# Rutgers-ECE-MML4SS/multimodal-sensor-fusion-with-attention-RajeevAtla

Measured on AMD Instinct MI355X. Metric: HybridFusion fwd+bwd samples/sec at 1/2/4/8 MI355X; CPU-ref parity, higher is better.
Workload: dtype fp32; 1 GPU; c2: HybridFusion M=3 B=256/gpu L=128 D=128 H=128 heads=4 C=5 dropout=0.1 train, fwd+CE(ls=0.05)+bwd+clip(1.0)+AdamW; fused step (flat buffers, one hipGraph); global_batch=256, per_gpu_batch=256, seq_len=128, parallelism=dp1, graph=True, matmul_precision=highest

## Files before the change

multimodal-sensor-fusion-with-attention-rajeevatla_amd/csrc/capi_util.h:

```cpp
#pragma once

#include <cstdarg>
#include <cstdio>
#include <cstring>
#include <string>
#include <vector>

#include "mmf_internal.h"
#include "mmfusion.h"

namespace mmf {

int fail(int code, const char* fmt, ...);

struct ProfRec { const char* name; hipEvent_t a, b; };
struct LaunchRec { const char* stage; const char* kernel; double flops, bytes; hipEvent_t a, b; };
struct Prof {
  bool on = false;
  const char* cur_stage = "";
  std::vector<ProfRec> recs;
  std::vector<LaunchRec> launches;
  std::vector<hipEvent_t> pool;
  size_t next = 0;
  hipEvent_t ev() {
    if (next == pool.size()) {
      hipEvent_t e;
      if (hipEventCreate(&e) != hipSuccess) return nullptr;
      pool.push_back(e);
    }
    return pool[next++];
  }
};
extern Prof g_prof;

// ... 79 lines not shown

inline void add_src(GemmJob& j, Operand a, Operand b, int K) {
  GemmSrc& s = j.src[j.nsrc++];
  s.a = a;
  s.b = b;
  s.K = K;
}

inline void split_rows(int rows, int& nsplit, int& kchunk, int hint = 0) {
  if (hint > 0) {
    kchunk = (rows + hint - 1) / hint;
    kchunk = (kchunk + 31) & ~31;
    nsplit = (rows + kchunk - 1) / kchunk;
    return;
  }
  int chunk = rows / 4;
  if (chunk > 512) chunk = 512;
  if (chunk < 64) chunk = 64;
  nsplit = (rows + chunk - 1) / chunk;
  if (nsplit < 1) nsplit = 1;
  if (nsplit > 64) nsplit = 64;
  kchunk = (rows + nsplit - 1) / nsplit;
  kchunk = (kchunk + 31) & ~31;
  nsplit = (rows + kchunk - 1) / kchunk;
}

inline size_t slab_bytes(int M, int N, int rows) {
  int nsplit, kchunk;
  split_rows(rows, nsplit, kchunk);
  return ((((size_t)nsplit * M * N * 4) + 255) & ~size_t(255)) +
         ((((size_t)nsplit * M * 4) + 255) & ~size_t(255)) + 256;
}

struct WgradPlan {
  std::vector<GemmJob> jobs;
  std::vector<ReduceJob> reds;
  int split_hint = 0;
  std::vector<GemmJob> jobs_b16;
  bool size_only = false;
};

inline void plan_wgrad(WgradPlan& wp, Bump& ws, int M, int N, int rows, Operand a, Operand b,
                       float* out_w, float* out_b, bool has_db, float alpha = 1.f) {
  int nsplit, kchunk;
  split_rows(rows, nsplit, kchunk, wp.split_hint);
  float* part = ws.take<float>((size_t)nsplit * M * N);
  float* part_db = has_db ? ws.take<float>((size_t)nsplit * M) : nullptr;
  GemmJob j = make_job(M, N, part, N, EPI_PARTIAL);
  j.g.alpha = alpha;
  j.g.nsplit = nsplit;
  j.g.kchunk = kchunk;
  j.g.part_db = part_db;
  if (wp.size_only) return;
  add_src(j, a, b, rows);
  wp.jobs.push_back(j);
  ReduceJob r;
  memset(&r, 0, sizeof(r));
  r.nbatch = 1;
  r.part = part;
  r.part_db = part_db;
  r.out = out_w;
  r.db = out_b;
  r.nsplit = nsplit;
  r.M = M;
  r.N = N;
  wp.reds.push_back(r);
}

inline void plan_wgrad_batched(WgradPlan& wp, Bump& ws, int M, int N, int rows, Operand a, Operand b,
                               float* out_w, int nbatch, int bs_a, int bs_b, int bs_out) {
  int nsplit, kchunk;
  split_rows(rows, nsplit, kchunk);
  float* part = ws.take<float>((size_t)nbatch * nsplit * M * N);
  GemmJob j = make_job(M, N, part, N, EPI_PARTIAL);
  j.g.nsplit = nsplit;
  j.g.kchunk = kchunk;
  j.g.nbatch = nbatch;
  j.g.bs_a = bs_a;
// ... 36 lines not shown
```

multimodal-sensor-fusion-with-attention-rajeevatla_amd/csrc/gemm.hip:

```cpp
#include <algorithm>
#include <cstdlib>
#include <cstring>
#include <map>
#include <vector>

#include "mmf_device.h"

namespace mmf {

namespace {

constexpr int BM = 128, BN = 128, BK = 32, NT = 256;
#ifndef MMF_GEMM_DK
#define MMF_GEMM_DK 16
#endif
#ifndef MMF_GEMM_NS
#define MMF_GEMM_NS 3
#endif
constexpr int LDS_STRIDE = BM + 4;
constexpr int LDS_STRIDE_T = BM + 1;

typedef float f32x4 __attribute__((ext_vector_type(4)));

struct TileCtx {
  int i0, j0, batch, split, nsplit;
  float* Cb;
  float* part_db;
  const float* biasb;
  int brs_off;
};

int gemm_interleave_mode() {
  const char* e = getenv("MMF_GEMM_ILV");
  if (!e || !e[0]) return 1;
  return e[0] == '0' ? 0 : (e[0] == '2' ? 2 : 1);
}
// ... 585 lines not shown
    __syncthreads();
    if (t >= BM) red[t - BM] = dbsum;
    __syncthreads();
    if (t < BM && T.i0 + t < G.M)
      T.part_db[(int64_t)T.split * G.M + T.i0 + t] = (dbsum + red[t]) * G.alpha;
  }
  if constexpr (WIDE) {
    f32x16 lo[2][2] = {{acc[0][0], acc[0][1]}, {acc[1][0], acc[1][1]}};
    epilogue<PR>(G, T, lo, lds, rs, p, inv_keep, wm, wn, h, c);
    TileCtx T2 = T;
    T2.j0 += BN;
    f32x16 hi[2][2] = {{acc[0][2], acc[0][3]}, {acc[1][2], acc[1][3]}};
    epilogue<PR>(G, T2, hi, lds, rs, p, inv_keep, wm, wn, h, c);
  } else {
    epilogue<PR>(G, T, acc, lds, rs, p, inv_keep, wm, wn, h, c);
  }
  if constexpr (!CHAIN) break;
  if (!G.chain) break;
  gi = G.chain - 1;
  asm volatile("s_waitcnt vmcnt(0)" ::: "memory");
  __syncthreads();
  __builtin_amdgcn_fence(__ATOMIC_ACQUIRE, "agent");
  }
}

template <int AMODE, int BMODE, int DK, int NSTAGE, int BF = 0, int B16 = 0, int WIDE = 0>
__global__ __launch_bounds__(NT, (NSTAGE * (B16 ? DK / 2 : DK) <= 32 ? 4 : 2)) void gemm_lds_kernel(const GemmArgs args) {
  gemm_lds_body<AMODE, BMODE, DK, NSTAGE, BF, B16, WIDE, 0>(args);
}
template <int AMODE, int BMODE, int DK, int NSTAGE, int BF = 0>
__global__ __launch_bounds__(NT) __attribute__((amdgpu_waves_per_eu(3)))
void gemm_lds_chain_kernel(const GemmArgs args) {
  gemm_lds_body<AMODE, BMODE, DK, NSTAGE, BF, 0, 0, 1>(args);
}

constexpr int WSR_DK = 16, WSR_NS = 6, WSR_NKC = 16;

template <int BF, bool EXT>
__global__ __launch_bounds__(NT, 2) void gemm_wsr_kernel(const GemmArgs args, int total_items, int K) {
  constexpr int DTILE = BM * WSR_DK;
  __shared__ __attribute__((aligned(16))) float ring[WSR_NS * DTILE];
  __shared__ float csx[BN];
  const int t = threadIdx.x;
  const int lane = t & 63, wave = t >> 6;
  const int h = lane >> 5, c = lane & 31;
  const int wm = wave >> 1, wn = wave & 1;
  const int nkt = K / WSR_DK, nkc = K / 8;

  RngSnap rs{0, 0};
  const float p = args.drop_p;
  const float inv_keep = p < 1.f ? 1.f / (1.f - p) : 0.f;
  const uint32_t thr = p16(p);
  if (p > 0.f && args.rng) rs = *args.rng;
  if (args.rng_advance && blockIdx.x == 0 && threadIdx.x == 0) args.rng_advance[1] += 1;
  const int nwg = gridDim.x;
  const int item0 = (int)(((int64_t)blockIdx.x * total_items) / nwg);
  const int item1 = (int)(((int64_t)(blockIdx.x + 1) * total_items) / nwg);
  if (item0 >= item1) return;

  const int nflat = (item1 - item0) * nkt;
  auto item_group = [&](int item, int& rowtile) {
    int g = 0;
#pragma unroll
    for (int i = 1; i < GEMM_MAX_GROUPS; ++i)
      if (i < args.ngroups && item >= args.tile_off[i]) g = i;
    rowtile = item - args.tile_off[g];
// ... 1018 lines not shown
        mmf_launch((KERNEL<MODE_KR, MODE_KR>), grid, dim3(NT), 0, st, args);       \
      else                                                                                 \
        mmf_launch((KERNEL<MODE_KR, MODE_RK>), grid, dim3(NT), 0, st, args);
      if (nch) {
        if (bmode == MODE_KR) {
          if (pr == 2) mmf_launch((gemm_lds_chain_kernel<MODE_RK, MODE_KR, 16, 3, 2>), grid, dim3(NT), 0, st, args);
          else if (pr == 1) mmf_launch((gemm_lds_chain_kernel<MODE_RK, MODE_KR, 16, 3, 1>), grid, dim3(NT), 0, st, args);
          else mmf_launch((gemm_lds_chain_kernel<MODE_RK, MODE_KR, 16, 3, 0>), grid, dim3(NT), 0, st, args);
        } else {
          if (pr == 2) mmf_launch((gemm_lds_chain_kernel<MODE_RK, MODE_RK, 16, 3, 2>), grid, dim3(NT), 0, st, args);
          else if (pr == 1) mmf_launch((gemm_lds_chain_kernel<MODE_RK, MODE_RK, 16, 3, 1>), grid, dim3(NT), 0, st, args);
          else mmf_launch((gemm_lds_chain_kernel<MODE_RK, MODE_RK, 16, 3, 0>), grid, dim3(NT), 0, st, args);
        }
      } else if (fast) {
        MMF_LAUNCH_CFG(MMF_GEMM_DK, MMF_GEMM_NS)
      } else {
        MMF_LAUNCH(gemm_generic_kernel)
      }
#undef MMF_LAUNCH
#undef MMF_LAUNCH_CFG
#undef MMF_LAUNCH_CFG2
      hipError_t e = hipGetLastError();
      if (e != hipSuccess) return e;
    } else if (args.rng_advance) {
      rng_advance = args.rng_advance;
    }
  }
  if (!later.empty())
    if (hipError_t e = launch_gemm(later.data(), (int)later.size(), amode, bmode, drop_p, rng, st, nullptr))
      return e;
  return left.finish(hipSuccess);
}

__global__ __launch_bounds__(256) void cvt_bf16_kernel(const CvtArgs a) {
  const int q = blockIdx.y;
  const float* s = a.src[q];
  __bf16* d = a.dst[q];
  const int64_t n = a.n[q];
  if (float* d32 = a.dst32[q]) {
    for (int64_t i = (int64_t)blockIdx.x * 256 + threadIdx.x; i < n; i += (int64_t)gridDim.x * 256) d32[i] = s[i];
    return;
  }
  for (int64_t i = 4 * ((int64_t)blockIdx.x * 256 + threadIdx.x); i < n; i += 4 * (int64_t)gridDim.x * 256) {
    if (i + 4 <= n) {
      const float4 v = *reinterpret_cast<const float4*>(s + i);
      d[i] = (__bf16)v.x; d[i + 1] = (__bf16)v.y; d[i + 2] = (__bf16)v.z; d[i + 3] = (__bf16)v.w;
    } else {
      for (int64_t e = i; e < n; ++e) d[e] = (__bf16)s[e];
    }
  }
}

hipError_t launch_cvt_bf16(const CvtArgs& a, hipStream_t st) {
  if (a.count <= 0) return hipSuccess;
  if (a.count > CVT_MAX) return hipErrorInvalidValue;
  int64_t mx = 0;
  double by = 0.0;
  for (int i = 0; i < a.count; ++i) {
    if (!a.dst32[i] && ((uintptr_t)a.src[i] & 15) != 0) return hipErrorInvalidValue;
    mx = std::max<int64_t>(mx, a.dst32[i] ? a.n[i] : a.n[i] / 4);
    by += (a.dst32[i] ? 8.0 : 6.0) * a.n[i];
  }
  const int gx = (int)std::min<int64_t>((mx + 255) / 256, 64);
  ProfLaunch prof_(st, "cvt_bf16_kernel", 0.0, by);
  mmf_launch(cvt_bf16_kernel, dim3(std::max(gx, 1), a.count), dim3(256), 0, st, a);
  return hipGetLastError();
// ... 269 lines not shown
```

multimodal-sensor-fusion-with-attention-rajeevatla_amd/csrc/hybrid.hip:

```cpp
#include <algorithm>
#include <cmath>
#include <cstdlib>
#include <cstdio>
#include <cstring>
#include <unistd.h>

#include "capi_util.h"

using namespace mmf;

namespace {

const char* const kPlanKnobs[] = {
    "MMF_PSTORE", "MMF_NO_LONG_FUSED", "MMF_NO_FUSED_BWD", "MMF_NO_BF16_QK", "MMF_NO_GEMM_B16",
    "MMF_QK_CAT", "MMF_NO_DQK_B16", "MMF_NO_PROJ_B16", "MMF_NO_PCOL", "MMF_NO_POOLE", "MMF_POOLE_FLAT",
    "MMF_NO_L1_LEAN", "MMF_WGRAD_SPLIT_CAP", "MMF_NO_SIDE_STREAM", "MMF_SIDE_STREAM", "MMF_KW_SERIAL",
    "MMF_KW_FUSED", "MMF_NO_KW_FUSED", "MMF_NO_GATE_B16", "MMF_POOL_PER_PAIR", "MMF_TAIL_S"};

uint32_t plan_flags_now() {
  uint32_t sum = 0;
  for (char** e = environ; e && *e; ++e) {
    const char* s = *e;
    if (std::strncmp(s, "MMF_", 4) != 0) continue;
    for (const char* k : kPlanKnobs) {
      const size_t n = std::strlen(k);
      if (std::strncmp(s, k, n) != 0 || s[n] != '=') continue;
      uint32_t h = 2166136261u;
      for (const char* c = s; *c; ++c) h = (h ^ (uint8_t)*c) * 16777619u;
      sum += h | 1u;
      break;
    }
  }
  return sum;
}

int check_buffers(const mmf_hybrid_desc* d, size_t need_saved, size_t need_ws) {
  const uint32_t now = plan_flags_now();
  if (d->plan_flags != now)
    return fail(MMF_EINVAL,
                "the plan switches (MMF_* environment) changed since this descriptor's buffers were sized "
                "(plan_flags %08x, now %08x): size the buffers again and set plan_flags = mmf_hybrid_plan_flags()",
                d->plan_flags, now);
  if (need_saved != ~size_t(0) && need_saved > d->saved_capacity)
    return fail(MMF_EINVAL, "saved buffer too small: this call's layout needs %zu bytes, saved_capacity is %llu",
                need_saved, (unsigned long long)d->saved_capacity);
  if (need_ws != ~size_t(0) && need_ws > d->workspace_capacity)
    return fail(MMF_EINVAL, "workspace too small: this call's layout needs %zu bytes, workspace_capacity is %llu",
                need_ws, (unsigned long long)d->workspace_capacity);
  return MMF_OK;
}
// ... 279 lines not shown
                d->num_heads);
  if (d->hidden % 4 != 0 || d->hidden > 1024)
    return fail(MMF_ELIMIT, "hidden_dim must be a multiple of 4 and <= 1024 (got %d)", d->hidden);
  if (d->num_classes < 1) return fail(MMF_EINVAL, "num_classes must be >= 1");
  if (d->num_pairs < 0 || d->num_pairs > d->num_modalities * (d->num_modalities - 1))
    return fail(MMF_EINVAL, "bad num_pairs %d", d->num_pairs);
  for (int m = 0; m < d->num_modalities; ++m) {
    if (d->in_dim[m] < 1) return fail(MMF_EINVAL, "in_dim[%d] must be >= 1", m);
    if (d->seq_len[m] < 0) return fail(MMF_EINVAL, "seq_len[%d] must be >= 0", m);
  }
  for (int g = 0; g < d->num_pairs; ++g) {
    const int q = d->pair_q[g], k = d->pair_k[g];
    if (q < 0 || k < 0 || q >= d->num_modalities || k >= d->num_modalities || q == k)
      return fail(MMF_EINVAL, "bad pair %d: (%d, %d)", g, q, k);
  }
  if (!(d->dropout >= 0.f && d->dropout < 1.f))
    return fail(MMF_EINVAL, "dropout must be in [0, 1) (got %g)", (double)d->dropout);
  for (int g = 0; g < d->num_pairs; ++g)
    if (wide_pair(d, g) && !wide_supported(d->batch, d->num_heads, Lm(d, d->pair_q[g]), Lm(d, d->pair_k[g])))
      return fail(MMF_ELIMIT, "head_dim %d: pair %d's (heads x Lq x Lk) score tensor is too large",
                  d->hidden / d->num_heads, g);
  return MMF_OK;
}

void plan_wgrads(const mmf_hybrid_desc* d, const float* const* x, const float* mask,
                 const float* dlogits, const Saved& s, const Ws& w, const mmf_hybrid_grads* G,
                 Bump& bw, WgradPlan& wp, int part = 0) {
  const bool want_pairs = part != 2, want_proj = part != 1;
  const int B = d->batch, M = d->num_modalities, H = d->hidden, C = d->num_classes;
  const int nh = d->num_heads, hd = H / nh;
  const bool pool = use_pool(d);
  static const mmf_hybrid_grads kNull = {};
  const mmf_hybrid_grads* g = G ? G : &kNull;
  const int kBigRows = 4096;
  int nbig = 0;
  for (int p = 0; p < d->num_pairs && want_pairs; ++p) {
    const int lq = Lm(d, d->pair_q[p]), lk = Lm(d, d->pair_k[p]);
    if (!pool) nbig += (B * lq >= kBigRows) + (B * lk >= kBigRows);
    if (!single_key(d, p)) nbig += (B * lq >= kBigRows) + (B * lk >= kBigRows);
  }
  for (int m = 0; m < M && want_proj; ++m) nbig += (B * Lm(d, m) >= kBigRows);
  const int slots = 3 * device_cu_count();
  const int rem = nbig % GEMM_MAX_GROUPS, nfull = nbig - rem;
  int bi = 0;
  auto hint = [&](int rows) {
    if (rows < kBigRows) return 0;
    const int per = bi++ < nfull ? GEMM_MAX_GROUPS : rem;
    int sp = slots / per;
    if (const char* e = getenv("MMF_WGRAD_SPLIT_CAP")) sp = std::min(sp, std::max(1, atoi(e)));
    return std::max(1, std::min(sp, 256));
  };
  if (want_pairs) {
    plan_wgrad(wp, bw, C, H, B, opnd(dlogits, C), opnd(s.h1, H), g->cls2.w, g->cls2.b);
    plan_wgrad(wp, bw, H, H, B, opnd(w.dz1, H), opnd(s.fused, H), g->cls1.w, g->cls1.b);
    for (int m = 0; m < M; ++m)
      plan_wgrad(wp, bw, 1, H, B, opnd(w.dscore ? w.dscore + m : nullptr, M),
                 opnd(s.pooled ? s.pooled + (size_t)m * H : nullptr, M * H), g->gate[m].w, g->gate[m].b);
  }
  for (int p = 0; p < d->num_pairs && want_pairs; ++p) {
    const int q = d->pair_q[p], k = d->pair_k[p];
    const int lq = Lm(d, q), lk = Lm(d, k);
    const float* cq = w.cvec ? w.cvec + (size_t)q * H : nullptr;
    if (pool) {
      plan_wgrad(wp, bw, H, H, B, opnd(cq, M * H), opnd(s.Ob[p], H), g->o[p].w, g->o[p].b);
      Operand dob = opnd(w.dOb[p], H), u = opnd(s.U[p], nh * H), rr = opnd(s.r[p], nh);
      dob.vec = u.vec = (hd % 4 == 0) && (H % 4 == 0);
      rr.vec = 0;
      plan_wgrad_batched(wp, bw, hd, H, B, dob, u, g->v[p].w, nh, hd, H, hd * H);
      plan_wgrad_batched(wp, bw, hd, 1, B, dob, rr, g->v[p].b, nh, hd, 1, hd);
    } else {
      wp.split_hint = hint(B * lq);
      plan_wgrad(wp, bw, H, H, B * lq, opnd(cq, M * H, lq), opnd(s.O[p], H), g->o[p].w, g->o[p].b,
                 1.f / (float)lq);
      wp.split_hint = hint(B * lk);
      plan_wgrad(wp, bw, H, H, B * lk, opnd(w.dV[p], H), opnd(s.P[k], H), g->v[p].w, g->v[p].b);
    }
    if (single_key(d, p)) {
      plan_zero(wp, H, H, g->q[p].w, g->q[p].b);
      plan_zero(wp, H, H, g->k[p].w, g->k[p].b);
      continue;
    }
    const bool b16 = dqk_b16_on(d);
    const float* pq = b16 ? reinterpret_cast<const float*>(s.Pb[q]) : s.P[q];
    const float* pk = b16 ? reinterpret_cast<const float*>(s.Pb[k]) : s.P[k];
    wp.split_hint = hint(B * lq);
    plan_wgrad(wp, bw, H, H, B * lq, opnd(w.dQ[p], s.ldq[p]), opnd(pq, H), g->q[p].w, g->q[p].b);
    if (b16 && !wp.size_only) { wp.jobs_b16.push_back(wp.jobs.back()); wp.jobs.pop_back(); }
    wp.split_hint = hint(B * lk);
    plan_wgrad(wp, bw, H, H, B * lk, opnd(w.dK[p], s.ldk[p]), opnd(pk, H), g->k[p].w, g->k[p].b);
    if (b16 && !wp.size_only) { wp.jobs_b16.push_back(wp.jobs.back()); wp.jobs.pop_back(); }
    wp.split_hint = 0;
  }
  for (int m = 0; m < M && want_proj; ++m) {
    const int L = Lm(d, m), D = d->in_dim[m];
    wp.split_hint = hint(B * L);
    plan_wgrad(wp, bw, H, D, B * L, opnd(w.dZ[m], H), opnd(s.Xd[m], D), g->proj[m].w, g->proj[m].b);
    if (proj_b16_on(d) && !wp.size_only) { wp.jobs_b16.push_back(wp.jobs.back()); wp.jobs.pop_back(); }
    wp.split_hint = 0;
  }
}

size_t saved_bytes(const mmf_hybrid_desc* d) {
  MathScope math_(d->matmul_precision);
  Bump bp(nullptr);
  Saved s{};
  layout_saved(d, bp, s);
  return bp.off + 256;
}

size_t workspace_bytes(const mmf_hybrid_desc* d) {
  MathScope math_(d->matmul_precision);
  Bump bs(nullptr);
  Saved s{};
  layout_saved(d, bs, s);
  Bump bw(nullptr);
  Ws w;
  layout_ws(d, bw, w);
  size_t top = 0;
  for (int part = 0; part < 3; ++part) {
    Bump b = bw;
    WgradPlan wp;
    wp.size_only = true;
    plan_wgrads(d, nullptr, nullptr, nullptr, s, w, nullptr, b, wp, part);
    top = std::max(top, b.off);
  }
  return top + 256;
}

void fill_head(HeadArgs& ha, const mmf_hybrid_desc* d, const mmf_hybrid_params* W, const float* mask,
               const Saved& s) {
  const bool pool = use_pool(d);
// ... 774 lines not shown
      for (int g = 0; g < d->num_pairs; ++g)
        if (d->pair_k[g] == m) {
          e.pbar[e.nsrc] = s.pbar[g];
          e.du[e.nsrc++] = w.dU[g];
        }
    }
    if (!em.empty()) STAGE_TRY("bwd.pool_e", launch_pool_e(em.data(), (int)em.size(), B, nh, H, st));
  } else if (d->num_pairs) {
    std::vector<GemmJob> jobs;
    for (int g = 0; g < d->num_pairs; ++g) {
      const int q = d->pair_q[g], lq = Lm(d, q);
      GemmJob j = make_job(B * lq, H, w.dO[g], H, 0);
      j.g.alpha = 1.f / (float)lq;
      add_src(j, opnd(w.cvec + (size_t)q * H, M * H, lq), opnd(W->o[g].w, H), H);
      jobs.push_back(j);
    }
    STAGE_TRY("bwd.out_dO_gemm", launch_gemm(jobs.data(), (int)jobs.size(), MODE_RK, MODE_KR, 0.f, rng, st));
    if (nmp) {
      STAGE_TRY("bwd.attn_prep", launch_attn_bwd_stage(0, pairs.data(), nmp, B, nh, hd, scale, p, rng, st));
      STAGE_TRY("bwd.attn_dkv", launch_attn_bwd_stage(1, pairs.data(), nmp, B, nh, hd, scale, p, rng, st));
      STAGE_TRY("bwd.attn_dq", launch_attn_bwd_stage(2, pairs.data(), nmp, B, nh, hd, scale, p, rng, st));
    }
    if (nsk) STAGE_TRY("bwd.attn_single_key_dv", launch_sk_dv(skp.data(), nsk, B, nh, hd, p, rng, st));
    if (nwp) STAGE_TRY("bwd.attn_wide", launch_wide_bwd(wpairs.data(), nwp, B, nh, hd, scale, p, rng, false, st));
  }
  }
  if (part == 1) {
    std::stable_sort(wp.jobs.begin(), wp.jobs.end(), [](const GemmJob& a, const GemmJob& b) {
      const int64_t wa = (int64_t)a.g.nsplit * std::max(1, a.g.nbatch) * a.g.M * a.g.N;
      const int64_t wb = (int64_t)b.g.nsplit * std::max(1, b.g.nbatch) * b.g.M * b.g.N;
      return wa > wb;
    });
    STAGE_TRY("bwd.wgrad_gemm", launch_gemm(wp.jobs.data(), (int)wp.jobs.size(), MODE_KR, MODE_KR, p, rng, st));
    if (!wp.jobs_b16.empty())
      STAGE_TRY("bwd.wgrad_gemm", launch_gemm_b16(wp.jobs_b16.data(), (int)wp.jobs_b16.size(), st, MODE_KR, MODE_KR));
    STAGE_TRY("bwd.wgrad_reduce", launch_reduce(wp.reds.data(), (int)wp.reds.size(), st));
    return MMF_OK;
  }
  std::vector<GemmJob> dxjobs(M);
  std::vector<bool> has_dx(M, false);
  const bool pb16 = proj_b16_on(d);
  for (int m = 0; m < M; ++m) {
    if (!dx || !dx[m]) continue;
    const int L = Lm(d, m), D = d->in_dim[m];
    GemmJob j = make_job(B * L, D, dx[m], D, EPI_ROWSCALE | (drop ? EPI_DROP : 0));
    j.g.rowscale = mask; j.g.rs_div = L; j.g.rs_stride = M; j.g.rs_off = m;
    j.g.drop_site = SITE_IN + m;
    add_src(j, opnd(w.dZ[m], H), opnd(pb16 ? reinterpret_cast<const float*>(s.Wpb[m]) : W->proj[m].w, D), H);
    dxjobs[m] = j;
    has_dx[m] = true;
  }
  const bool chain_dx = !dqk_b16_on(d) && !pb16 && getenv("MMF_DX_CHAIN");
  {
    std::vector<GemmJob> jobs;
    for (int m = 0; m < M; ++m) {
      const int L = Lm(d, m);
      const bool pe = pool && poole_in_dz(d, m);
      GemmJob j = make_job(B * L, H, w.dZ[m], H,
                           EPI_GATE | (pool && !pe ? EPI_ADDMAT : EPI_ROWADD) | (proj_b16_on(d) ? EPI_BF16 : 0));
      if (pool && !pe) {
        j.g.addm = w.E[m];
        j.g.ld_addm = H;
      } else {
        j.g.rowadd = w.cvec + (size_t)m * H;
        j.g.ld_rowadd = M * H;
        j.g.rowadd_div = L;
// ... 23 lines not shown
        }
      }
      if (pe) {
        j.g.seg_rows = L;
        for (int g = 0; g < d->num_pairs; ++g)
          if (d->pair_k[g] == m && j.nsrc < GEMM_MAX_SRCS) {
            Operand du = opnd(w.dU[g], H);
            du.seg_stride = nh * H;
            add_src(j, opnd(s.pbarT[g], nh), du, nh);
          }
      }
      if (j.nsrc > GEMM_MAX_SRCS) return fail(MMF_ELIMIT, "too many gradient sources");
      if (chain_dx && has_dx[m]) j.chain = &dxjobs[m];
      jobs.push_back(j);
    }
    if (dqk_b16_on(d)) STAGE_TRY("bwd.dZ_gemm", launch_gemm_b16(jobs.data(), (int)jobs.size(), st, MODE_RK, MODE_KR));
    else STAGE_TRY("bwd.dZ_gemm", launch_gemm(jobs.data(), (int)jobs.size(), MODE_RK, MODE_KR, chain_dx ? p : 0.f, rng, st));
  }
  if (!chain_dx) {
    std::vector<GemmJob> jobs;
    for (int m = 0; m < M; ++m)
      if (has_dx[m]) jobs.push_back(dxjobs[m]);
    if (!jobs.empty() && pb16)
      STAGE_TRY("bwd.dx_gemm", launch_gemm_b16(jobs.data(), (int)jobs.size(), st, MODE_RK, MODE_KR, p, rng));
    else if (!jobs.empty())
      STAGE_TRY("bwd.dx_gemm", launch_gemm(jobs.data(), (int)jobs.size(), MODE_RK, MODE_KR, p, rng, st));
  }
  std::stable_sort(wp.jobs.begin(), wp.jobs.end(), [](const GemmJob& a, const GemmJob& b) {
    const int64_t wa = (int64_t)a.g.nsplit * std::max(1, a.g.nbatch) * a.g.M * a.g.N;
    const int64_t wb = (int64_t)b.g.nsplit * std::max(1, b.g.nbatch) * b.g.M * b.g.N;
    return wa > wb;
  });
  STAGE_TRY("bwd.wgrad_gemm", launch_gemm(wp.jobs.data(), (int)wp.jobs.size(), MODE_KR, MODE_KR, p, rng, st));
  if (!wp.jobs_b16.empty())
    STAGE_TRY("bwd.wgrad_gemm", launch_gemm_b16(wp.jobs_b16.data(), (int)wp.jobs_b16.size(), st, MODE_KR, MODE_KR));
  STAGE_TRY("bwd.wgrad_reduce", launch_reduce(wp.reds.data(), (int)wp.reds.size(), st));
  return MMF_OK;
}

int mmf_hybrid_backward(const mmf_hybrid_desc* d, const mmf_hybrid_params* W, const float* const* x,
                        const float* mask, const void* saved, const float* dlogits, void* workspace,
                        const mmf_hybrid_grads* G, float* const* dx, void* stream) {
  return hybrid_backward(d, W, x, mask, saved, dlogits, workspace, G, dx, stream, false);
}

uint32_t mmf_hybrid_plan_flags(void) { return plan_flags_now(); }

int mmf_hybrid_lean_l1(const mmf_hybrid_desc* d) {
  if (check_hybrid(d) != MMF_OK) return 0;
  return lean_l1_desc(d) ? 1 : 0;
}

size_t mmf_hybrid_train_sync_bytes(const mmf_hybrid_desc* d) {
  if (check_hybrid(d) != MMF_OK) return 0;
  const size_t tiles = ((size_t)d->batch + 15) / 16;
  return std::max<size_t>(256, (4 * (tiles * (3 + L1_MAXM) + 1) + 255) / 256 * 256);
}

int mmf_hybrid_train_status(const mmf_hybrid_desc* d, void* sync, int clear, void* stream) {
  const int rc = check_hybrid(d);
  if (rc) return rc;
  if (!sync) return fail(MMF_EINVAL, "train status: null sync buffer");
  const size_t tiles = ((size_t)d->batch + 15) / 16;
  uint32_t* err = static_cast<uint32_t*>(sync) + tiles * (3 + L1_MAXM);
  hipStream_t st = (hipStream_t)stream;
  uint32_t v = 0;
// ... 97 lines not shown
```

multimodal-sensor-fusion-with-attention-rajeevatla_amd/csrc/mmf_internal.h:

```cpp
#pragma once

#include <hip/hip_runtime.h>
#include <hip/hip_ext.h>
#include <stdint.h>
#include <stddef.h>

namespace mmf {

struct RngSnap { uint64_t seed; uint64_t offset; };

struct ProfArm {
  hipEvent_t a = nullptr, b = nullptr;
  int launches = 0;
};
extern thread_local ProfArm* g_prof_arm;
bool prof_arm_begin(ProfArm& arm, hipStream_t st);
bool prof_capturing(hipStream_t st);

struct SideStream { hipStream_t s; hipEvent_t fork_ev, join_ev; };
SideStream* side_stream(bool create);
void prof_arm_end(ProfArm& arm, hipStream_t st, const char* kernel, double flops, double bytes);
struct ProfLaunch {
  hipStream_t st;
  const char* kernel;
// ... 54 lines not shown
};

enum : int32_t {
  EPI_BIAS = 1, EPI_RELU = 2, EPI_DROP = 4, EPI_ROWADD = 8, EPI_GATE = 16,
  EPI_ROWSCALE = 32, EPI_PARTIAL = 64, EPI_BIAS_RS = 128, EPI_ADDMAT = 256,
  EPI_COLSUM = 512,
  EPI_BF16 = 1024,
  EPI_BF16COPY = 2048,
  EPI_GATE_B16 = 4096
};

struct GemmGroup {
  int32_t M, N;
  int32_t src_begin, src_count;
  float* C; int32_t ldc;
  int32_t epi;
  float alpha;
  const float* bias;
  const float* bias_rs; int32_t bias_rs_ld, bias_rs_off;
  const float* addm; int32_t ld_addm;
  float rowadd_scale;
  const float* rowadd; int32_t ld_rowadd, rowadd_div;
  const float* gate; int32_t ld_gate; float gate_scale;
  const float* rowscale; int32_t rs_div, rs_stride;
  int32_t rs_off;
  uint32_t drop_site;
  int32_t nsplit, kchunk;
  union { float* part_db; float* colsum; };
  int32_t nbatch;
  int32_t bs_a, bs_b, bs_c, bs_bias, bs_brs;
  int32_t seg_rows;
  void* copy;
  int32_t chain;
};

constexpr int GEMM_MAX_GROUPS = 32;
constexpr int GEMM_MAX_SRCS = 32;

struct GemmArgs {
  GemmGroup g[GEMM_MAX_GROUPS];
  GemmSrc s[GEMM_MAX_SRCS];
  int32_t tile_off[GEMM_MAX_GROUPS];
  int32_t ngroups;
  int32_t amode, bmode;
  float drop_p;
  const RngSnap* rng;
  uint64_t* rng_advance;
  int32_t ilv;
};

struct GemmJob {
  GemmGroup g;
  GemmSrc src[GEMM_MAX_SRCS];
  int nsrc;
  const GemmJob* chain;
};

hipError_t launch_gemm(const GemmJob* jobs, int njobs, int amode, int bmode, float drop_p,
                       const RngSnap* rng, hipStream_t st, uint64_t* rng_advance = nullptr);
int device_cu_count();

struct MaskDropJob {
  const float* x; float* out;
  int64_t rows; int32_t D, L;
  uint32_t site; int32_t vec, outb;
};
struct MaskDropArgs {
  MaskDropJob j[8];
  int32_t n, M;
  const float* mask;
  float p;
  const RngSnap* rng;
  const uint64_t* rng_live;
  RngSnap* rng_snap;
  struct KeepWordJob { uint32_t* bits; uint32_t Lq, Lk, kw_ld, site; } kw[16];
  int32_t nkw, B, heads;
};
hipError_t launch_mask_dropout(MaskDropArgs a, hipStream_t st);

struct ReduceJob {
  const float* part; const float* part_db;
  float* out; float* db;
  int32_t nsplit, M, N;
  int32_t nbatch, bs_out, bs_db;
};
hipError_t launch_gemm_b16(const GemmJob* jobs, int njobs, hipStream_t st, int amode = MODE_RK, int bmode = MODE_RK,
                           float drop_p = 0.f, const RngSnap* rng = nullptr, uint64_t* rng_advance = nullptr);
constexpr int CVT_MAX = 72;
struct CvtArgs {
  const float* src[CVT_MAX]; __bf16* dst[CVT_MAX]; float* dst32[CVT_MAX]; int64_t n[CVT_MAX]; int32_t count;
};
hipError_t launch_cvt_bf16(const CvtArgs& a, hipStream_t st);
bool gemm_b16_ok(const GemmJob& J, int amode = MODE_RK, int bmode = MODE_RK);
// ... 290 lines not shown
```

Measured before the change: 273,800 samples/s.

## Add paired wide-K wgrad GEMM kernel sharing the B operand across jobs

Adds a dedicated fp32 weight-gradient GEMM kernel that, for Q/K/projection wgrad jobs sharing the same right-hand operand (P or X), stages both A operands plus one shared B tile per K step. This lets one workgroup compute two 128x128 partials, and it folds the bias column sums into the same pass. A new planner picks one K-chunk size so the total number of workgroups fits about two per CU, moves eligible jobs into a separate launch, and tags unpaired jobs so they split their chunk into two halves. The aim is fewer redundant B loads and fewer split partials to reduce, which should mean fewer workgroups and a lighter reduce pass. In exchange it adds a large new code path with more register pressure (launch bound of 2 waves) and more planning complexity.

```diff
diff --git a/multimodal-sensor-fusion-with-attention-rajeevatla_amd/csrc/capi_util.h b/multimodal-sensor-fusion-with-attention-rajeevatla_amd/csrc/capi_util.h
--- a/multimodal-sensor-fusion-with-attention-rajeevatla_amd/csrc/capi_util.h
+++ b/multimodal-sensor-fusion-with-attention-rajeevatla_amd/csrc/capi_util.h
@@ -1,5 +1,6 @@
 #pragma once
 
+#include <algorithm>
 #include <cstdarg>
 #include <cstdio>
 #include <cstring>
@@ -145,18 +146,38 @@
          ((((size_t)nsplit * M * 4) + 255) & ~size_t(255)) + 256;
 }
 
+inline int wide_kchunk(const std::vector<int>& fat_rows, const std::vector<int>& single_rows, int slots) {
+  int maxr = 64;
+  for (int r : fat_rows) maxr = std::max(maxr, r);
+  for (int r : single_rows) maxr = std::max(maxr, (r + 1) / 2);
+  for (int kc = 64; kc < maxr; kc += 32) {
+    long wgs = 0;
+    for (int r : fat_rows) wgs += (r + kc - 1) / kc;
+    for (int r : single_rows) wgs += (r + 2 * kc - 1) / (2 * kc);
+    if (wgs <= slots) return kc;
+  }
+  return (maxr + 31) & ~31;
+}
+
 struct WgradPlan {
   std::vector<GemmJob> jobs;
   std::vector<ReduceJob> reds;
   int split_hint = 0;
+  int kchunk_hint = 0;
   std::vector<GemmJob> jobs_b16;
+  std::vector<GemmJob> jobs_wide;
   bool size_only = false;
 };
 
 inline void plan_wgrad(WgradPlan& wp, Bump& ws, int M, int N, int rows, Operand a, Operand b,
                        float* out_w, float* out_b, bool has_db, float alpha = 1.f) {
   int nsplit, kchunk;
-  split_rows(rows, nsplit, kchunk, wp.split_hint);
+  if (wp.kchunk_hint > 0) {
+    kchunk = wp.kchunk_hint;
+    nsplit = (rows + kchunk - 1) / kchunk;
+  } else {
+    split_rows(rows, nsplit, kchunk, wp.split_hint);
+  }
   float* part = ws.take<float>((size_t)nsplit * M * N);
   float* part_db = has_db ? ws.take<float>((size_t)nsplit * M) : nullptr;
   GemmJob j = make_job(M, N, part, N, EPI_PARTIAL);
diff --git a/multimodal-sensor-fusion-with-attention-rajeevatla_amd/csrc/gemm.hip b/multimodal-sensor-fusion-with-attention-rajeevatla_amd/csrc/gemm.hip
--- a/multimodal-sensor-fusion-with-attention-rajeevatla_amd/csrc/gemm.hip
+++ b/multimodal-sensor-fusion-with-attention-rajeevatla_amd/csrc/gemm.hip
@@ -2,6 +2,7 @@
 #include <cstdlib>
 #include <cstring>
 #include <map>
+#include <type_traits>
 #include <vector>
 
 #include "mmf_device.h"
@@ -653,6 +654,187 @@
 __global__ __launch_bounds__(NT) __attribute__((amdgpu_waves_per_eu(3)))
 void gemm_lds_chain_kernel(const GemmArgs args) {
   gemm_lds_body<AMODE, BMODE, DK, NSTAGE, BF, 0, 0, 1>(args);
+}
+
+template <int AMODE, int BMODE, int DK, int NSTAGE, int BF = 0>
+__global__ __launch_bounds__(NT, 2) void gemm_lds_wa_kernel(const GemmArgs args) {
+  static_assert(AMODE == MODE_KR && BMODE == MODE_KR && BF == 0, "fp32 KR x KR form only");
+  constexpr int DTILE = BM * DK;
+  constexpr int SSTRIDE = 3 * DTILE;
+  constexpr int PT = BM * DK / 256 / 4;
+  __shared__ __attribute__((aligned(16))) float lds[NSTAGE * SSTRIDE + 2 * BM];
+  static_assert(NSTAGE * SSTRIDE >= 64 * CS, "epilogue image does not fit");
+  static_assert(NSTAGE == 3, "ring depth (the wait counts below)");
+
+  int local;
+  const int gi = group_of_block(args, local);
+  const GemmGroup& G = args.g[gi];
+  TileCtx T;
+  if (!tile_ctx(G, local, T)) return;
+  const bool two = G.pair > 0, halves = G.pair < 0;
+  const GemmGroup& G2 = args.g[two ? G.pair - 1 : gi];
+
+  const int t = threadIdx.x;
+  const int lane = t & 63, wave = __builtin_amdgcn_readfirstlane(t >> 6);
+  const int h = lane >> 5, c = lane & 31;
+  const int wm = wave >> 1, wn = wave & 1;
+
+  auto operand = [](const Operand& o) { return Operand{o.ptr, o.ld, 1, 1, 0}; };
+  const Operand opA = operand(args.s[G.src_begin].a), opB = operand(args.s[G.src_begin].b),
+                opA2 = operand(args.s[G2.src_begin].a);
+  const int64_t offA = (int64_t)T.batch * G.bs_a, offB = (int64_t)T.batch * G.bs_b;
+  const int kbeg = T.split * G.kchunk;
+  const int kend = min(args.s[G.src_begin].K, kbeg + G.kchunk);
+  const int ntiles = kend > kbeg ? (kend - kbeg + DK - 1) / DK : 0;
+
+  f32x16 acc[2][2][2];
+#pragma unroll
+  for (int q = 0; q < 2; ++q)
+#pragma unroll
+    for (int a = 0; a < 2; ++a)
+#pragma unroll
+      for (int b = 0; b < 2; ++b)
+#pragma unroll
+        for (int r = 0; r < 16; ++r) acc[q][a][b][r] = 0.f;
+  float dbs[2][2] = {{0.f, 0.f}, {0.f, 0.f}};
+  float dbp = 0.f;
+
+  auto main_loop = [&](auto two_c) {
+    constexpr bool TWO = decltype(two_c)::value;
+    auto stage = [&](int buf, int k0) {
+      float* At = lds + buf * SSTRIDE;
+      stage_tile<MODE_KR, DK>(At, opA, offA, T.i0, G.M, k0, kend, wave, lane);
+      if constexpr (TWO) stage_tile<MODE_KR, DK>(At + DTILE, opA2, 0, T.i0, G.M, k0, kend, wave, lane);
+      stage_tile<MODE_KR, DK>(At + 2 * DTILE, opB, offB, T.j0, G.N, k0, kend, wave, lane);
+    };
+    int nissued = 0;
+    for (; nissued < NSTAGE - 1 && nissued < ntiles; ++nissued) stage(nissued, kbeg + nissued * DK);
+    int buf = 0, tile = 0;
+    auto k_tile = [&](auto set_c) {
+      constexpr int Q = decltype(set_c)::value;
+      if (nissued - tile - 1 <= 0) asm volatile("s_waitcnt vmcnt(0)" ::: "memory");
+      else asm volatile("s_waitcnt vmcnt(%0)" ::"n"((TWO ? 3 : 2) * PT) : "memory");
+      lds_barrier();
+      float* A1 = lds + buf * SSTRIDE;
+      float* A2 = A1 + DTILE;
+      float* Bt = A1 + 2 * DTILE;
+      const int kv = kend - (kbeg + tile * DK);
+      if (kv < DK) {
+        zero_tail<MODE_KR, DK>(A1, kv);
+        if constexpr (TWO) zero_tail<MODE_KR, DK>(A2, kv);
+        zero_tail<MODE_KR, DK>(Bt, kv);
+        lds_barrier();
+      }
+      f32x4 bf[DK / 8][2], a1[DK / 8][2], a2[DK / 8][2];
+#pragma unroll
+      for (int j = 0; j < DK / 8; ++j) {
+#pragma unroll
+        for (int b = 0; b < 2; ++b) bf[j][b] = frag<MODE_KR, DK>(Bt, wn * 64 + b * 32 + c, j, h);
+#pragma unroll
+        for (int a = 0; a < 2; ++a) {
+          a1[j][a] = frag<MODE_KR, DK>(A1, wm * 64 + a * 32 + c, j, h);
+          if constexpr (TWO) a2[j][a] = frag<MODE_KR, DK>(A2, wm * 64 + a * 32 + c, j, h);
+        }
+      }
+      __builtin_amdgcn_sched_barrier(0);
+      if constexpr (!TWO) {
+        if (!halves && T.part_db) {
+#pragma unroll
+          for (int q = 0; q < DK / 2; ++q) dbp += A1[((t >> 7) * (DK / 2) + q) * BM + (t & (BM - 1))];
+        }
+      }
+#pragma unroll
+      for (int j = 0; j < DK / 8; ++j) {
+        if (j == 1 && nissued < ntiles) {
+          stage(nissued % NSTAGE, kbeg + nissued * DK);
+          ++nissued;
+        }
+#pragma unroll
+        for (int a = 0; a < 2; ++a) {
+          dbs[Q][a] += (a1[j][a][0] + a1[j][a][1]) + (a1[j][a][2] + a1[j][a][3]);
+          if constexpr (TWO) dbs[1][a] += (a2[j][a][0] + a2[j][a][1]) + (a2[j][a][2] + a2[j][a][3]);
+        }
+#pragma unroll
+        for (int s = 0; s < 4; ++s)
+#pragma unroll
+          for (int a = 0; a < 2; ++a)
+#pragma unroll
+            for (int b = 0; b < 2; ++b) {
+              acc[Q][a][b] = mfma32(a1[j][a][s], bf[j][b][s], acc[Q][a][b]);
+              if constexpr (TWO) acc[1][a][b] = mfma32(a2[j][a][s], bf[j][b][s], acc[1][a][b]);
+            }
+      }
+      buf = buf == NSTAGE - 1 ? 0 : buf + 1;
+      ++tile;
+    };
+    if constexpr (TWO) {
+      while (tile < ntiles) k_tile(std::integral_constant<int, 0>{});
+    } else {
+      const int nh = halves ? min(ntiles, max(1, G.kchunk / (2 * DK))) : ntiles;
+      while (tile < nh) k_tile(std::integral_constant<int, 0>{});
+      while (tile < ntiles) k_tile(std::integral_constant<int, 1>{});
+    }
+  };
+  if (two) {
+    main_loop(std::true_type{});
+  } else {
+    main_loop(std::false_type{});
+#pragma unroll
+    for (int a = 0; a < 2; ++a) {
+      dbs[0][a] += dbs[1][a];
+#pragma unroll
+      for (int b = 0; b < 2; ++b) acc[0][a][b] += acc[1][a][b];
+    }
+  }
+
+  {
+    float* red = lds + NSTAGE * SSTRIDE;
+    const int row = wm * 64 + wn * 32 + c;
+    const float d0 = wn ? dbs[0][1] : dbs[0][0], d1 = wn ? dbs[1][1] : dbs[1][0];
+    if (!two && !halves) {
+      if (t >= BM) red[t - BM] = dbp;
+    } else if (h == 1) {
+      red[row] = d0;
+      red[BM + row] = d1;
+    }
+    __syncthreads();
+    if (!two && !halves) {
+      if (t < BM && t < G.M && T.part_db) T.part_db[(int64_t)T.split * G.M + t] = (dbp + red[t]) * G.alpha;
+    } else if (h == 0 && row < G.M) {
+      if (T.part_db) T.part_db[(int64_t)T.split * G.M + row] = (d0 + red[row]) * G.alpha;
+      if (two && G2.part_db) G2.part_db[(int64_t)T.split * G2.M + row] = (d1 + red[BM + row]) * G2.alpha;
+    }
+  }
+  auto store_half = [&](const GemmGroup& Gq, float* Cb, const f32x16 (&hacc)[2][2]) {
+    float* const out = Cb + (int64_t)T.split * Gq.M * BN;
+    const float alpha = Gq.alpha;
+    const int cg = (t & 15) * 8;
+#pragma unroll
+    for (int pass = 0; pass < 2; ++pass) {
+      __syncthreads();
+      if (wm == pass) {
+#pragma unroll
+        for (int a = 0; a < 2; ++a)
+#pragma unroll
+          for (int b = 0; b < 2; ++b)
+#pragma unroll
+            for (int r = 0; r < 16; ++r) lds[(a * 32 + acc_row(r, h)) * CS + wn * 64 + b * 32 + c] = hacc[a][b][r];
+      }
+      __syncthreads();
+#pragma unroll
+      for (int it = 0; it < 4; ++it) {
+        const int lr = (t >> 4) + 16 * it;
+        if (pass * 64 + lr >= Gq.M) continue;
+        const f32x4 lo = *reinterpret_cast<const f32x4*>(lds + lr * CS + cg);
+        const f32x4 hi = *reinterpret_cast<const f32x4*>(lds + lr * CS + cg + 4);
+        float* o = out + (int64_t)(pass * 64 + lr) * BN + cg;
+        *reinterpret_cast<f32x4*>(o) = lo * alpha;
+        *reinterpret_cast<f32x4*>(o + 4) = hi * alpha;
+      }
+    }
+  };
+  store_half(G, T.Cb, acc[0]);
+  if (two) store_half(G2, G2.C, acc[1]);
 }
 
 constexpr int WSR_DK = 16, WSR_NS = 6, WSR_NKC = 16;
@@ -1737,6 +1919,101 @@
   return left.finish(hipSuccess);
 }
 
+bool wgrad_wide_on() {
+  const char* e = getenv("MMF_WGRAD_WIDE");
+  return !(e && e[0] == '0');
+}
+
+bool wgrad_wide_job(const GemmJob& J) {
+  const GemmGroup& g = J.g;
+  if (math_mode() != 0 || J.nsrc != 1 || J.chain || g.epi != EPI_PARTIAL) return false;
+  const int nb = g.nbatch < 1 ? 1 : g.nbatch;
+  if (g.M < 4 || g.M > BM || g.M % 4 != 0 || g.N != BN || g.seg_rows > 0 || g.nsplit < 1) return false;
+  if (nb > 1 && g.part_db) return false;
+  if (g.part_db && ((uintptr_t)g.part_db & 3) != 0) return false;
+  if (g.kchunk < MMF_GEMM_DK || g.kchunk % MMF_GEMM_DK != 0) return false;
+  const GemmSrc& s = J.src[0];
+  if (((uintptr_t)g.C & 15) != 0) return false;
+  if (s.K % 4 != 0 || g.kchunk % 32 != 0) return false;
+  return s.K >= 1 && s.a.row_div == 1 && s.b.row_div == 1 && s.a.seg_stride == 0 && s.b.seg_stride == 0 &&
+         dma_ok(s.a, MODE_KR, g.M, g.bs_a, nb) && dma_ok(s.b, MODE_KR, g.N, g.bs_b, nb);
+}
+
+hipError_t launch_gemm_wa(const GemmJob* jobs, int njobs, hipStream_t st) {
+  std::vector<GemmJob> rest;
+  std::vector<int> order;
+  for (int i = 0; i < njobs; ++i) {
+    if (wgrad_wide_job(jobs[i])) order.push_back(i);
+    else rest.push_back(jobs[i]);
+  }
+  std::stable_sort(order.begin(), order.end(), [&](int x, int y) {
+    const GemmJob &a = jobs[x], &b = jobs[y];
+    const int wa = std::min(a.g.kchunk, a.src[0].K), wb = std::min(b.g.kchunk, b.src[0].K);
+    if ((wa >= 256) != (wb >= 256)) return wa >= 256;
+    if (a.src[0].b.ptr != b.src[0].b.ptr) return a.src[0].b.ptr < b.src[0].b.ptr;
+    return a.g.kchunk < b.g.kchunk;
+  });
+  auto partners = [&](const GemmJob& a, const GemmJob& b) {
+    if (a.g.M != BM || b.g.M != BM || a.g.nbatch > 1 || b.g.nbatch > 1) return false;
+    return a.src[0].b.ptr == b.src[0].b.ptr && a.src[0].b.ld == b.src[0].b.ld && a.src[0].K == b.src[0].K &&
+           a.g.kchunk == b.g.kchunk && a.g.nsplit == b.g.nsplit && a.g.alpha == b.g.alpha;
+  };
+  size_t done = 0;
+  while (done < order.size()) {
+    GemmArgs args;
+    memset(&args, 0, sizeof(args));
+    args.amode = args.bmode = MODE_KR;
+    int ng = 0, np = 0, max_blocks = 0;
+    const GemmJob* second[GEMM_MAX_GROUPS];
+    double fl = 0.0, by = 0.0;
+    while (done < order.size()) {
+      const GemmJob& J = jobs[order[done]];
+      const bool two = done + 1 < order.size() && partners(J, jobs[order[done + 1]]);
+      if (ng + np + (two ? 2 : 1) > GEMM_MAX_GROUPS) break;
+      GemmGroup g = J.g;
+      if (g.nbatch < 1) g.nbatch = 1;
+      g.src_count = 1;
+      g.chain = 0;
+      g.pair = (!two && J.g.pair < 0) ? -1 : 0;
+      g.src_begin = ng;
+      args.s[ng] = J.src[0];
+      second[ng] = two ? &jobs[order[done + 1]] : nullptr;
+      np += two ? 1 : 0;
+      args.tile_off[ng] = max_blocks;
+      args.g[ng++] = g;
+      max_blocks += g.nsplit * g.nbatch;
+      const double K = (double)J.src[0].K * g.nbatch;
+      fl += 2.0 * g.M * g.N * K * (two ? 2 : 1);
+      by += 4.0 * ((two ? 2.0 : 1.0) * g.M + g.N) * K + 4.0 * (two ? 2 : 1) * g.nsplit * g.nbatch * g.M * g.N;
+      done += two ? 2 : 1;
+    }
+    int nx = ng;
+    for (int gi = 0; gi < ng; ++gi) {
+      if (!second[gi]) continue;
+      GemmGroup g = second[gi]->g;
+      g.nbatch = 1;
+      g.src_begin = nx;
+      g.src_count = 1;
+      g.chain = 0;
+      g.pair = 0;
+      args.s[nx] = second[gi]->src[0];
+      args.tile_off[nx] = max_blocks;
+      args.g[nx] = g;
+      args.g[gi].pair = nx + 1;
+      ++nx;
+    }
+    args.ngroups = nx;
+    if (max_blocks > 0) {
+      ProfLaunch prof_(st, "gemm_lds_wa_kernel<1, 1, 16, 3, 0>", fl, by);
+      mmf_launch((gemm_lds_wa_kernel<MODE_KR, MODE_KR, MMF_GEMM_DK, 3, 0>), dim3(max_blocks, 1), dim3(NT), 0, st, args);
+      const hipError_t e = hipGetLastError();
+      if (e != hipSuccess) return e;
+    }
+  }
+  if (!rest.empty()) return launch_gemm(rest.data(), (int)rest.size(), MODE_KR, MODE_KR, 0.f, nullptr, st);
+  return hipSuccess;
+}
+
 __global__ __launch_bounds__(256) void cvt_bf16_kernel(const CvtArgs a) {
   const int q = blockIdx.y;
   const float* s = a.src[q];
diff --git a/multimodal-sensor-fusion-with-attention-rajeevatla_amd/csrc/hybrid.hip b/multimodal-sensor-fusion-with-attention-rajeevatla_amd/csrc/hybrid.hip
--- a/multimodal-sensor-fusion-with-attention-rajeevatla_amd/csrc/hybrid.hip
+++ b/multimodal-sensor-fusion-with-attention-rajeevatla_amd/csrc/hybrid.hip
@@ -15,7 +15,7 @@
     "MMF_PSTORE", "MMF_NO_LONG_FUSED", "MMF_NO_FUSED_BWD", "MMF_NO_BF16_QK", "MMF_NO_GEMM_B16",
     "MMF_QK_CAT", "MMF_NO_DQK_B16", "MMF_NO_PROJ_B16", "MMF_NO_PCOL", "MMF_NO_POOLE", "MMF_POOLE_FLAT",
     "MMF_NO_L1_LEAN", "MMF_WGRAD_SPLIT_CAP", "MMF_NO_SIDE_STREAM", "MMF_SIDE_STREAM", "MMF_KW_SERIAL",
-    "MMF_KW_FUSED", "MMF_NO_KW_FUSED", "MMF_NO_GATE_B16", "MMF_POOL_PER_PAIR", "MMF_TAIL_S"};
+    "MMF_KW_FUSED", "MMF_NO_KW_FUSED", "MMF_NO_GATE_B16", "MMF_POOL_PER_PAIR", "MMF_TAIL_S", "MMF_WGRAD_WIDE"};
 
 uint32_t plan_flags_now() {
   uint32_t sum = 0;
@@ -361,14 +361,55 @@
   const bool pool = use_pool(d);
   static const mmf_hybrid_grads kNull = {};
   const mmf_hybrid_grads* g = G ? G : &kNull;
+  const bool b16 = dqk_b16_on(d), pb16 = proj_b16_on(d);
+  const bool wide = wgrad_wide_on() && math_mode() == 0 && H == 128 && !b16;
+  auto qk_wide = [&](int p) {
+    return wide && !single_key(d, p) && s.ldq[p] % 4 == 0 && s.ldk[p] % 4 == 0;
+  };
+  auto proj_wide = [&](int m) { return wide && !pb16 && d->in_dim[m] == 128; };
+  int wkey_n[2 * MMF_MAX_MODALITIES] = {}, wkey_i[2 * MMF_MAX_MODALITIES] = {};
+  for (int p = 0; p < d->num_pairs && want_pairs; ++p)
+    if (qk_wide(p)) { ++wkey_n[d->pair_q[p]]; ++wkey_n[d->pair_k[p]]; }
+  for (int m = 0; m < M && want_proj; ++m)
+    if (proj_wide(m)) ++wkey_n[M + m];
+  int wkc = 0;
+  {
+    std::vector<int> fat, single;
+    for (int key = 0; key < 2 * M; ++key) {
+      const int rows = B * Lm(d, key % M);
+      for (int i = 0; i < wkey_n[key] / 2; ++i) fat.push_back(rows);
+      if (wkey_n[key] & 1) single.push_back(rows);
+    }
+    if (!fat.empty() || !single.empty()) wkc = wide_kchunk(fat, single, 2 * device_cu_count());
+  }
+  bool last_paired = false;
+  auto wide_chunk = [&](int key, int rows) {
+    const bool paired = wkey_i[key] < (wkey_n[key] & ~1);
+    last_paired = paired;
+    ++wkey_i[key];
+    int kc = paired ? wkc : 2 * wkc;
+    if (const char* e = getenv("MMF_WGRAD_SPLIT_CAP")) {
+      const int cap = std::max(1, atoi(e));
+      kc = std::max(kc, (((rows + cap - 1) / cap) + 31) & ~31);
+    }
+    return kc;
+  };
+  auto take_wide = [&]() {
+    wp.kchunk_hint = 0;
+    if (wp.size_only) return;
+    wp.jobs_wide.push_back(wp.jobs.back());
+    wp.jobs.pop_back();
+    wp.jobs_wide.back().g.pair = last_paired ? 0 : -1;
+  };
   const int kBigRows = 4096;
   int nbig = 0;
   for (int p = 0; p < d->num_pairs && want_pairs; ++p) {
     const int lq = Lm(d, d->pair_q[p]), lk = Lm(d, d->pair_k[p]);
     if (!pool) nbig += (B * lq >= kBigRows) + (B * lk >= kBigRows);
-    if (!single_key(d, p)) nbig += (B * lq >= kBigRows) + (B * lk >= kBigRows);
-  }
-  for (int m = 0; m < M && want_proj; ++m) nbig += (B * Lm(d, m) >= kBigRows);
+    if (!single_key(d, p) && !qk_wide(p)) nbig += (B * lq >= kBigRows) + (B * lk >= kBigRows);
+  }
+  for (int m = 0; m < M && want_proj; ++m)
+    if (!proj_wide(m)) nbig += (B * Lm(d, m) >= kBigRows);
   const int slots = 3 * device_cu_count();
   const int rem = nbig % GEMM_MAX_GROUPS, nfull = nbig - rem;
   int bi = 0;
@@ -409,23 +450,35 @@
       plan_zero(wp, H, H, g->k[p].w, g->k[p].b);
       continue;
     }
-    const bool b16 = dqk_b16_on(d);
     const float* pq = b16 ? reinterpret_cast<const float*>(s.Pb[q]) : s.P[q];
     const float* pk = b16 ? reinterpret_cast<const float*>(s.Pb[k]) : s.P[k];
-    wp.split_hint = hint(B * lq);
+    const bool wq = qk_wide(p);
+    if (wq) wp.kchunk_hint = wide_chunk(q, B * lq);
+    else wp.split_hint = hint(B * lq);
     plan_wgrad(wp, bw, H, H, B * lq, opnd(w.dQ[p], s.ldq[p]), opnd(pq, H), g->q[p].w, g->q[p].b);
+    if (wq) take_wide();
     if (b16 && !wp.size_only) { wp.jobs_b16.push_back(wp.jobs.back()); wp.jobs.pop_back(); }
-    wp.split_hint = hint(B * lk);
+    if (wq) wp.kchunk_hint = wide_chunk(k, B * lk);
+    else wp.split_hint = hint(B * lk);
     plan_wgrad(wp, bw, H, H, B * lk, opnd(w.dK[p], s.ldk[p]), opnd(pk, H), g->k[p].w, g->k[p].b);
+    if (wq) take_wide();
     if (b16 && !wp.size_only) { wp.jobs_b16.push_back(wp.jobs.back()); wp.jobs.pop_back(); }
     wp.split_hint = 0;
   }
   for (int m = 0; m < M && want_proj; ++m) {
     const int L = Lm(d, m), D = d->in_dim[m];
-    wp.split_hint = hint(B * L);
+    const bool wm = proj_wide(m);
+    if (wm) wp.kchunk_hint = wide_chunk(M + m, B * L);
+    else wp.split_hint = hint(B * L);
     plan_wgrad(wp, bw, H, D, B * L, opnd(w.dZ[m], H), opnd(s.Xd[m], D), g->proj[m].w, g->proj[m].b);
-    if (proj_b16_on(d) && !wp.size_only) { wp.jobs_b16.push_back(wp.jobs.back()); wp.jobs.pop_back(); }
+    if (wm) take_wide();
+    if (pb16 && !wp.size_only) { wp.jobs_b16.push_back(wp.jobs.back()); wp.jobs.pop_back(); }
     wp.split_hint = 0;
+  }
+  if (!wp.jobs_wide.empty()) {
+    std::vector<GemmJob> keep;
+    for (const GemmJob& j : wp.jobs) (wgrad_wide_job(j) ? wp.jobs_wide : keep).push_back(j);
+    wp.jobs.swap(keep);
   }
 }
 
@@ -1266,6 +1319,8 @@
       return wa > wb;
     });
     STAGE_TRY("bwd.wgrad_gemm", launch_gemm(wp.jobs.data(), (int)wp.jobs.size(), MODE_KR, MODE_KR, p, rng, st));
+    if (!wp.jobs_wide.empty())
+      STAGE_TRY("bwd.wgrad_gemm", launch_gemm_wa(wp.jobs_wide.data(), (int)wp.jobs_wide.size(), st));
     if (!wp.jobs_b16.empty())
       STAGE_TRY("bwd.wgrad_gemm", launch_gemm_b16(wp.jobs_b16.data(), (int)wp.jobs_b16.size(), st, MODE_KR, MODE_KR));
     STAGE_TRY("bwd.wgrad_reduce", launch_reduce(wp.reds.data(), (int)wp.reds.size(), st));
@@ -1355,6 +1410,8 @@
     return wa > wb;
   });
   STAGE_TRY("bwd.wgrad_gemm", launch_gemm(wp.jobs.data(), (int)wp.jobs.size(), MODE_KR, MODE_KR, p, rng, st));
+  if (!wp.jobs_wide.empty())
+    STAGE_TRY("bwd.wgrad_gemm", launch_gemm_wa(wp.jobs_wide.data(), (int)wp.jobs_wide.size(), st));
   if (!wp.jobs_b16.empty())
     STAGE_TRY("bwd.wgrad_gemm", launch_gemm_b16(wp.jobs_b16.data(), (int)wp.jobs_b16.size(), st, MODE_KR, MODE_KR));
   STAGE_TRY("bwd.wgrad_reduce", launch_reduce(wp.reds.data(), (int)wp.reds.size(), st));
diff --git a/multimodal-sensor-fusion-with-attention-rajeevatla_amd/csrc/mmf_internal.h b/multimodal-sensor-fusion-with-attention-rajeevatla_amd/csrc/mmf_internal.h
--- a/multimodal-sensor-fusion-with-attention-rajeevatla_amd/csrc/mmf_internal.h
+++ b/multimodal-sensor-fusion-with-attention-rajeevatla_amd/csrc/mmf_internal.h
@@ -110,6 +110,7 @@
   int32_t seg_rows;
   void* copy;
   int32_t chain;
+  int32_t pair;
 };
 
 constexpr int GEMM_MAX_GROUPS = 32;
@@ -137,6 +138,9 @@
 hipError_t launch_gemm(const GemmJob* jobs, int njobs, int amode, int bmode, float drop_p,
                        const RngSnap* rng, hipStream_t st, uint64_t* rng_advance = nullptr);
 int device_cu_count();
+bool wgrad_wide_on();
+bool wgrad_wide_job(const GemmJob& J);
+hipError_t launch_gemm_wa(const GemmJob* jobs, int njobs, hipStream_t st);
 
 struct MaskDropJob {
   const float* x; float* out;
```

Measured after the change: 275,800 samples/s, median of 6. Within noise of the previous version (+0.7%).
